# Dunni3/keypoint-diffusion

Measured on AMD Instinct MI355X. Metric: denoising steps/sec, higher is better.
Workload: dtype f32; 1 GPU; egnn_all_atom dynamics (6 EGNN layers, hidden 256, update_kp_feat; fixed receptor encoder), batch of 64 synthetic 300-atom pockets / 25-atom ligands per GPU, T=500, seeded random-init weights, every step taken from the t=T ligand state; batch_per_gpu=64, n_rec=300, n_lig=25, parallelism=dp1

## Files before the change

include/kpd.h:

```cpp
#ifndef KPD_H
#define KPD_H

#include <stdint.h>

#ifdef __cplusplus
extern "C" {
#endif

typedef enum kpd_status {
    KPD_OK = 0,
    KPD_ERR_INVALID = -1,
    KPD_ERR_CAPACITY = -2,
    KPD_ERR_WEIGHTS = -3,
    KPD_ERR_HIP = -4,
    KPD_ERR_STATE = -5
} kpd_status;

const char *kpd_last_error(void);
int kpd_version(void);
int kpd_build_flags(void);

typedef struct kpd_batch {
    int32_t B;
    int32_t n_lig, n_kp;
// ... 16 lines not shown
    int32_t *ll_src, *ll_dst, *ll_rowptr;
    int32_t *kl_src, *kl_dst, *kl_rowptr;
    int32_t *lk_src, *lk_dst, *lk_rowptr;
    int32_t *ll_per_graph;
    int32_t *counts;
} kpd_lig_graph;

kpd_status kpd_build_lig_graph(const kpd_batch *batch, float ll_cutoff, int32_t ll_k, float kl_cutoff,
                               int32_t kl_k, const kpd_lig_graph *out, void *stream);

typedef struct kpd_egnn_config {
    int32_t atom_nf, rec_nf;
    int32_t n_layers, hidden_nf;
    int32_t use_tanh, norm, update_kp_feat;
    float message_norm;
    int32_t ll_k, kl_k;
    float ll_cutoff, kl_cutoff;
    float coords_range;
} kpd_egnn_config;

typedef struct kpd_egnn kpd_egnn;

kpd_status kpd_egnn_create(const kpd_egnn_config *cfg, kpd_egnn **out);
void kpd_egnn_destroy(kpd_egnn *m);
kpd_status kpd_egnn_load_weight(kpd_egnn *m, const char *name, const float *w_dev,
                                const int64_t *shape, int32_t ndim, void *stream);
kpd_status kpd_egnn_commit(kpd_egnn *m);
kpd_status kpd_egnn_reserve(kpd_egnn *m, int32_t max_B, int32_t max_n_lig, int32_t max_n_kp,
                            int32_t max_n_kk, int32_t max_lig_per_graph, int32_t max_kp_per_graph);
kpd_status kpd_egnn_forward(kpd_egnn *m, const kpd_batch *batch, const float *t_dev,
                            float *eps_h_dev, float *eps_x_dev, void *stream);
kpd_status kpd_egnn_debug_state(kpd_egnn *m, const char *what, float *out_dev, int64_t n_floats,
                                void *stream);
kpd_status kpd_egnn_profile(kpd_egnn *m, int32_t enable);
kpd_status kpd_egnn_profile_read(kpd_egnn *m, double *total_ms, int32_t *launches);
kpd_status kpd_egnn_last_counts(kpd_egnn *m, int32_t out[8], void *stream);

typedef struct kpd_egnn_trainer kpd_egnn_trainer;
kpd_status kpd_egnn_trainer_create(const kpd_egnn_config *cfg, kpd_egnn_trainer **out);
void kpd_egnn_trainer_destroy(kpd_egnn_trainer *t);
kpd_status kpd_egnn_trainer_bind(kpd_egnn_trainer *t, const char *name, const float *weight_dev, float *grad_dev,
                                 const int64_t *shape, int32_t ndim);
kpd_status kpd_egnn_trainer_reserve(kpd_egnn_trainer *t, int32_t max_B, int32_t max_n_lig, int32_t max_n_kp,
                                    int32_t max_n_kk, int32_t max_lig_per_graph, int32_t max_kp_per_graph);
kpd_status kpd_egnn_trainer_forward(kpd_egnn_trainer *t, const kpd_batch *batch, const float *t_dev, float *eps_h_dev,
                                    float *eps_x_dev, void *stream);
kpd_status kpd_egnn_trainer_backward(kpd_egnn_trainer *t, const float *d_eps_h, const float *d_eps_x, float *d_lig_h,
                                     float *d_lig_x, float *d_kp_h, float *d_kp_x, void *stream);
kpd_status kpd_egnn_trainer_profile(kpd_egnn_trainer *t, int32_t enable);
kpd_status kpd_egnn_trainer_profile_read(kpd_egnn_trainer *t, double total_ms[2], int32_t launches[2], double edges[2]);

typedef struct kpd_gvp_config {
    int32_t n_lig_scalars, n_kp_scalars;
    int32_t vector_size;
    int32_t n_convs, n_hidden_scalars;
    int32_t update_kp;
    int32_t message_norm_mode;
    float message_norm;
    int32_t ll_k, kl_k;
    float ll_cutoff, kl_cutoff;
    int32_t n_message_gvps, n_update_gvps, n_noise_gvps;
} kpd_gvp_config;

typedef struct kpd_gvp kpd_gvp;

kpd_status kpd_gvp_create(const kpd_gvp_config *cfg, kpd_gvp **out);
// ... 273 lines not shown
```

keypoint-diffusion_amd/csrc/egnn.hip:

```cpp
#include <string.h>

#include <map>
#include <set>
#include <string>
#include <vector>

#include "egnn_kernels.h"
#include "egnn_wide.h"
#include "mfma_core.h"

using namespace kpd;

namespace {

struct LayerW {
    float *wp_e[4], *wx_e[4], *b_e[4], *wr_e[4], *watt[4];
    float *wp_c[4], *wx_c[4], *b_c[4], *wr_c[4], *w3[4];
    void *wh_e[4], *wh_c[4];
    void *chh_p[2][NSLOT];
    void *wh_a[2], *wh_b[2], *wh_2[2];
    float *wp_p[2][NSLOT], *wx_p[2][NSLOT], *b_p[2][NSLOT];
    float *ch_p[2][NSLOT], *wcol_p[2][NSLOT];
    float *wp_a[2], *wx_a[2], *wp_b[2], *wx_b[2], *b0[2], *wp_2[2], *wx_2[2], *b2[2], *ln_w[2], *ln_b[2];
};
// ... 33 lines not shown
struct kpd_egnn {
    kpd_egnn_config cfg;
    int n_et;
    int n_upd;
    bool rec_identity;
    Arena warena, ws;
    std::vector<LayerW> L;
    float *le_W0, *le_b0, *le_W1t, *le_b1;
    float *re_W0, *re_b0, *re_W1t, *re_b1;
    float *de_W0, *de_b0, *de_W1, *de_b1;
    std::set<std::string> expected, loaded;
    bool committed = false;
    int debug_layers = -1;
    bool f16_ok = true;
    float *widen_buf = nullptr;
    int *widen_map = nullptr;
    size_t widen_floats = 0, widen_ints = 0;
    int gemm_mode = 0;
    bool f32_only = false;
    int prune_last = 1;
    bool prof_on = false;
    std::vector<hipEvent_t> prof_ev;
    size_t prof_used = 0;

    int cap_B = 0, cap_lig = 0, cap_kp = 0, cap_kk = 0, cap_ll = 0, cap_kl = 0, cap_maxlig = 0, cap_maxkp = 0;
    int tile_cap = 0, tiles_et_cap[4] = {0, 0, 0, 0};
    float *h[2], *x[2], *P[2];
    float *hn_main[4], *hn_cont[4], *xn_main[4], *xn_cont[4];
    int *bidx[2];
    float *z[2];
    int *meta, *ll_deg, *ll_off, *kl_off, *kl_pg;
    kpd_lig_graph lg;
    int kp_table = 1;
    int tab_rows = 0;
    bool last_table = false;
    int *rowmap = nullptr, *kp_ok = nullptr;
    float *tab_in = nullptr;
    int *tab_bidx = nullptr;
    float *hT = nullptr, *PT = nullptr;
    EgnnWide *wide = nullptr;
};

static kpd_status build_weight_arena(kpd_egnn *m) {
    const kpd_egnn_config &c = m->cfg;
    m->warena.poison_at = 2;
    m->L.assign(c.n_layers, LayerW());
    return carve(m->warena, ARENA_TAIL, [&](Carve &A) {
        for (int i = 0; i < c.n_layers; ++i) {
            LayerW &w = m->L[i];
            const std::string pre = "egnn.conv_layers." + std::to_string(i) + ".";
            for (int et = 0; et < m->n_et; ++et) {
                A(w.wp_e[et], WP_FLOATS); A(w.wx_e[et], HS); A(w.b_e[et], HS); A(w.wr_e[et], HS); A(w.watt[et], HS);
                A(w.wp_c[et], WP_FLOATS); A(w.wx_c[et], HS); A(w.b_c[et], HS); A(w.wr_c[et], HS); A(w.w3[et], HS);
                A.as<unsigned short>(w.wh_e[et], WH_HALVES); A.as<unsigned short>(w.wh_c[et], WH_HALVES);
                for (int var = 0; var < 2; ++var) {
                    const int ss = kSrcSlot[et] + var, ds = kDstSlot[et] + var;
                    A(w.wp_p[kSrcNt[et]][ss], WP_FLOATS); A(w.wx_p[kSrcNt[et]][ss], HS);
                    A(w.wp_p[kDstNt[et]][ds], WP_FLOATS); A(w.wx_p[kDstNt[et]][ds], HS); A(w.b_p[kDstNt[et]][ds], HS);
                    A(w.ch_p[kSrcNt[et]][ss], 16 * 4096); A(w.wcol_p[kSrcNt[et]][ss], HS);
                    A(w.ch_p[kDstNt[et]][ds], 16 * 4096); A(w.wcol_p[kDstNt[et]][ds], HS);
                    A.as<unsigned short>(w.chh_p[kSrcNt[et]][ss], CHH_HALVES);
                    A.as<unsigned short>(w.chh_p[kDstNt[et]][ds], CHH_HALVES);
                }
                const std::string e = kEtName[et];
                for (const char *blk : {"edge_mlp.", "coord_mlp."})
                    for (const char *s : {".0.weight", ".0.bias", ".2.weight", ".2.bias"}) m->expected.insert(pre + blk + e + s);
// ... 473 lines not shown
    const int n_layers = m->debug_layers >= 0 ? std::min(m->debug_layers, c.n_layers) : c.n_layers;

    auto slot_mask = [&](int etmask, int nt) {
        int mk = 0;
        for (int et = 0; et < 4; ++et)
            if ((etmask >> et) & 1) {
                if (kSrcNt[et] == nt) mk |= 3 << kSrcSlot[et];
                if (kDstNt[et] == nt) mk |= 3 << kDstSlot[et];
            }
        return mk;
    };
    auto layer_etmask = [&](int li) { return li == n_layers - 1 ? active_last : active; };
    for (int li = 0; li < n_layers; ++li) {
        const LayerW &L = m->L[li];
        {
            {
                ProjPair pp;
                memset(&pp, 0, sizeof(pp));
                for (int nt = 0; nt < 2; ++nt) {
                    ProjArgs &pa = pp.nt[nt];
                    pa.h = m->h[nt]; pa.n = n[nt]; pa.P = m->P[nt];
                    int k = 0;
                    const int mk = slot_mask(layer_etmask(li), nt);
                    for (int s = 0; s < NSLOT; ++s)
                        if (L.wp_p[nt][s] && ((mk >> s) & 1)) {
                            pa.wp[k] = L.wp_p[nt][s]; pa.wx[k] = L.wx_p[nt][s]; pa.bias[k] = L.b_p[nt][s]; pa.slot[k] = s;
                            pa.chain[k] = L.ch_p[nt][s]; pa.wcol[k] = L.wcol_p[nt][s]; pa.chain_h[k] = L.chh_p[nt][s];
                            ++k;
                        }
                    pp.n_slots[nt] = k;
                }
                pp.tiles0 = cdiv(n[0], TM);
                pp.gemm_mode = m->gemm_mode;
                if (kp_tab && li == 0) {
                    ProjPair pk = pp;
                    pk.n_slots[NT_LIG] = 0;
                    pk.skip_if = m->kp_ok;
                    ProjArgs &pa = pp.nt[NT_KP];
                    pa.h = m->hT; pa.n = n_tab; pa.P = m->PT;
                    KPD_TRY(launch_proj_chain(pp, st));
                    KPD_TRY(launch_proj_chain(pk, st));
                } else {
                    KPD_TRY(launch_proj_chain(pp, st));
                }
            }
        }
        EdgeArgs ea;
        memset(&ea, 0, sizeof(ea));
        const bool last = li == n_layers - 1;
        ea.meta = last ? m->meta + 16 : m->meta;
        ea.x[0] = x_cur[0]; ea.x[1] = x_cur[1]; ea.P[0] = m->P[0]; ea.P[1] = m->P[1];
        ea.use_tanh = c.use_tanh; ea.coords_range = c.coords_range;
        ea.tile_rows = tr;
        ea.gemm_mode = tr == TM ? m->gemm_mode : 0;
        for (int et = 0; et < 4; ++et) {
            ea.src[et] = esrc[et]; ea.dst[et] = edst[et];
            ea.src_nt[et] = kSrcNt[et]; ea.dst_nt[et] = kDstNt[et]; ea.src_slot[et] = kSrcSlot[et]; ea.dst_slot[et] = kDstSlot[et];
            ea.wr_e[et] = L.wr_e[et]; ea.wr_c[et] = L.wr_c[et];
            ea.wp_e[et] = L.wp_e[et]; ea.wx_e[et] = L.wx_e[et]; ea.b_e[et] = L.b_e[et];
            ea.wp_c[et] = L.wp_c[et]; ea.wx_c[et] = L.wx_c[et]; ea.b_c[et] = L.b_c[et];
            ea.wh_e[et] = L.wh_e[et]; ea.wh_c[et] = L.wh_c[et];
            ea.watt[et] = L.watt[et]; ea.w3[et] = L.w3[et];
            ea.hn_main[et] = m->hn_main[et]; ea.hn_cont[et] = m->hn_cont[et];
            ea.xn_main[et] = m->xn_main[et]; ea.xn_cont[et] = m->xn_cont[et];
        }
        if (kp_tab && li == 0) { ea.PT = m->PT; ea.rowmap = m->rowmap; ea.kp_ok = m->kp_ok; }
// ... 47 lines not shown
    KPD_TRY(launch_decode(m->h[NT_LIG], m->x[NT_LIG], bt->lig_x, bt->n_lig, c.atom_nf, 2 * c.atom_nf, m->de_W0, m->de_b0,
                          m->de_W1, m->de_b1, eps_h, eps_x, st));
    return KPD_OK;
}

extern "C" kpd_status kpd_egnn_debug_state(kpd_egnn *m, const char *what, float *out, int64_t n_floats, void *stream) {
    KPD_REQUIRE(m && what && out, KPD_ERR_INVALID, "null argument");
    hipStream_t st = static_cast<hipStream_t>(stream);
    if (m->wide) return wide_debug_state(m->wide, what, out, n_floats, st);
    const std::string w(what);
    const float *src = nullptr;
    if (w == "h_lig") src = m->h[0];
    else if (w == "h_kp") src = m->h[1];
    else if (w == "x_lig") src = m->x[0];
    else if (w == "x_kp") src = m->x[1];
    else if (w == "z_lig") src = m->z[0];
    else if (w == "z_kp") src = m->z[1];
    else if (w.size() == 4 && (w.rfind("xnm", 0) == 0 || w.rfind("xnc", 0) == 0 || w.rfind("hnm", 0) == 0 || w.rfind("hnc", 0) == 0) &&
             w[3] >= '0' && w[3] < '4') {
        const int et = w[3] - '0';
        src = w[0] == 'x' ? (w[2] == 'm' ? m->xn_main[et] : m->xn_cont[et]) : (w[2] == 'm' ? m->hn_main[et] : m->hn_cont[et]);
    }
    else if (w == "kp_table_ok") {
        KPD_REQUIRE(n_floats == 1, KPD_ERR_INVALID, "kp_table_ok is one value");
        if (!m->last_table) {
            KPD_HIP(hipMemsetAsync(out, 0, 4, st));
            return KPD_OK;
        }
        src = reinterpret_cast<const float *>(m->kp_ok);
    } else if (w.rfind("kp_table=", 0) == 0) {
        m->kp_table = atoi(w.c_str() + 9);
        return KPD_OK;
    }
    else if (w.rfind("layers=", 0) == 0) {
        m->debug_layers = atoi(w.c_str() + 7);
        return KPD_OK;
    } else if (w.rfind("prune=", 0) == 0) {
        m->prune_last = atoi(w.c_str() + 6);
        return KPD_OK;
    } else if (w.rfind("gemm=", 0) == 0) {
        const std::string v = w.substr(5);
        KPD_REQUIRE(v == "f32" || v == "f16x2", KPD_ERR_INVALID, "gemm mode must be f32 or f16x2");
        KPD_REQUIRE(v == "f32" || !m->f32_only, KPD_ERR_INVALID,
                    "gemm=f16x2: atom_nf = %d / rec_nf = %d (hidden_nf = %d) run the exact fp32 path only; the f16x2 mode covers atom_nf <= 32 "
                    "with rec_nf <= 128 or 256, or the identity keypoint encoder at hidden_nf 256", m->cfg.atom_nf, m->cfg.rec_nf, m->cfg.hidden_nf);
        KPD_REQUIRE(v == "f32" || !m->committed || m->f16_ok, KPD_ERR_WEIGHTS, "%s", F16_RANGE_ERROR);
        m->gemm_mode = v == "f16x2" ? 1 : 0;
        return KPD_OK;
    }
    KPD_REQUIRE(src, KPD_ERR_INVALID, "unknown debug tap '%s'", what);
    KPD_HIP(hipMemcpyAsync(out, src, (size_t)n_floats * 4, hipMemcpyDeviceToDevice, st));
    return KPD_OK;
}

extern "C" kpd_status kpd_egnn_profile(kpd_egnn *m, int32_t enable) {
    KPD_REQUIRE(m, KPD_ERR_INVALID, "null handle");
    KPD_REQUIRE(!m->wide, KPD_ERR_INVALID, "kpd_egnn_profile times the fused edge kernel of hidden_nf <= 256; hidden_nf = %d has none",
                m->cfg.hidden_nf);
    if (enable && m->prof_ev.empty()) {
        m->prof_ev.resize(2 * 8192);
        for (hipEvent_t &e : m->prof_ev) KPD_HIP(hipEventCreate(&e));
    }
    m->prof_on = enable != 0;
    m->prof_used = 0;
    return KPD_OK;
}
// ... 49 lines not shown
```

keypoint-diffusion_amd/csrc/egnn_chain.hip:

```cpp
#include <algorithm>
#include <cstdlib>

#include "chain_core.h"
#include "egnn_kernels.h"

namespace kpd {

namespace {

constexpr int ENT = 16;
constexpr int ECH4 = ENT * 64;

__device__ __forceinline__ float reduce_q(float v) {
    v += __shfl_xor(v, 16);
    v += __shfl_xor(v, 32);
    return v;
}

}

struct ProjWs {
    ProjPair p;
    int blocks0;
    int bpc[2];
    int tpb;
};

constexpr int WS_TILE = 128;
constexpr int WS_W4 = 16 * 8 * 64;
constexpr int WS_LDS_BYTES = WS_W4 * 16 + (128 + 128 + HS) * 4;

__global__ __launch_bounds__(512, 1) void k_proj_ws(ProjWs qa) {
    extern __shared__ __attribute__((aligned(16))) float smem[];
    v4f *W = reinterpret_cast<v4f *>(smem);
    float *s_wcol = smem + WS_W4 * 4, *s_bias = s_wcol + 128, *s_wrow = s_bias + 128;
    const int tid = threadIdx.x, wave = tid >> 6, lane = tid & 63;
    if (qa.p.skip_if && *qa.p.skip_if) return;
    const int which = (int)blockIdx.x >= qa.blocks0 ? 1 : 0;
    const ProjArgs &a = qa.p.nt[which];
    const int local = blockIdx.x - (which ? qa.blocks0 : 0);
    const int combo = local / qa.bpc[which], chunk = local - combo * qa.bpc[which];
    const int s = combo >> 1, hf = combo & 1;
    const int tiles = (a.n + WS_TILE - 1) / WS_TILE;
    const int t0 = chunk * qa.tpb, t1 = min(tiles, t0 + qa.tpb);
    if (t0 >= t1) return;
    {
        const v4f *src = reinterpret_cast<const v4f *>(a.chain[s]);
#pragma unroll
        for (int j = 0; j < WS_W4 / 512; ++j) {
            const int i = tid + 512 * j, ks = i >> 9, rem = i & 511;
            W[i] = src[(size_t)ks * ECH4 + 8 * hf * 64 + rem];
        }
        const float *bias = a.bias[s];
        if (tid < 128) {
            s_wcol[tid] = a.wcol[s][128 * hf + tid];
            s_bias[tid] = bias ? bias[128 * hf + tid] : 0.0f;
        }
        for (int i = tid; i < HS; i += 512) s_wrow[i] = i <= 256 ? a.wx[s][i] : 0.0f;
    }
    __syncthreads();
    const int el = lane & 15, q = lane >> 4;
    const float bias256 = a.bias[s] ? a.bias[s][256] : 0.0f;
    auto load_x = [&](int t, v4f (&x)[ENT], float &x256) {
        const int row = min(t * WS_TILE + 16 * wave + el, a.n - 1);
        const float *hrow = a.h + (size_t)row * HS;
#pragma unroll
        for (int nt = 0; nt < ENT; ++nt) x[nt] = *reinterpret_cast<const v4f *>(hrow + 16 * nt + 4 * q);
        x256 = hrow[256];
    };
    auto store_tile = [&](const v4f (&acc)[8], int row, float out256) {
        if (row >= 0 && row < a.n) {
            float *orow = a.P + ((size_t)row * NSLOT + a.slot[s]) * HS + 128 * hf;
#pragma unroll
            for (int m = 0; m < 8; ++m) *reinterpret_cast<v4f *>(orow + 16 * m + 4 * q) = acc[m];
            if (hf == 0 && q == 0) orow[256] = out256;
        }
    };
    v4f x[ENT], xn[ENT], accp[8];
    float h256, h256n, out256p = 0.0f;
    int rowp = -1;
#pragma unroll
    for (int m = 0; m < 8; ++m) accp[m] = zero4();
    load_x(t0, xn, h256n);
#pragma unroll 1
    for (int t = t0; t < t1; ++t) {
#pragma unroll
        for (int nt = 0; nt < ENT; ++nt)
#pragma unroll
            for (int r = 0; r < 4; ++r) asm volatile("v_mov_b32 %0, %1" : "=v"(x[nt][r]) : "v"(xn[nt][r]));
        asm volatile("v_mov_b32 %0, %1" : "=v"(h256) : "v"(h256n));
        __builtin_amdgcn_sched_barrier(0);
        store_tile(accp, rowp, out256p);
        if (t + 1 < t1) load_x(t + 1, xn, h256n);
        v4f acc[8];
#pragma unroll
        for (int m = 0; m < 8; ++m)
            acc[m] = h256 * *reinterpret_cast<const v4f *>(s_wcol + 16 * m + 4 * q) + *reinterpret_cast<const v4f *>(s_bias + 16 * m + 4 * q);
        float part = 0.0f;
        if (hf == 0) {
#pragma unroll
            for (int nt = 0; nt < ENT; ++nt) {
                const v4f wv = *reinterpret_cast<const v4f *>(s_wrow + 16 * nt + 4 * q);
                part += x[nt][0] * wv[0] + x[nt][1] * wv[1] + x[nt][2] * wv[2] + x[nt][3] * wv[3];
            }
        }
        const v4f *wp = W + lane;
        v4f w[2][4];
#pragma unroll
        for (int m = 0; m < 4; ++m) w[0][m] = wp[m * 64];
#pragma unroll
        for (int b = 0; b < 32; ++b) {
            if (b + 1 < 32) {
#pragma unroll
                for (int m = 0; m < 4; ++m) w[(b + 1) & 1][m] = wp[(4 * (b + 1) + m) * 64];
            }
            __builtin_amdgcn_sched_barrier(0);
            const v4f xin = x[b >> 1];
            const int g = b & 1;
#pragma unroll
            for (int r = 0; r < 4; ++r)
#pragma unroll
                for (int m = 0; m < 4; ++m) acc[4 * g + m] = mfma16(w[b & 1][m][r], xin[r], acc[4 * g + m]);
            __builtin_amdgcn_sched_barrier(0);
        }
        const int row = t * WS_TILE + 16 * wave + el;
        const float out256 = hf == 0 ? reduce_q(part) + bias256 + h256 * s_wrow[256] : 0.0f;
#pragma unroll
        for (int m = 0; m < 8; ++m) accp[m] = acc[m];
        rowp = row;
        out256p = out256;
    }
    store_tile(accp, rowp, out256p);
}

__global__ __launch_bounds__(512, 1) void k_proj_ws_h(ProjWs qa) {
    extern __shared__ __attribute__((aligned(16))) float smem[];
    f32x4 *W = reinterpret_cast<f32x4 *>(smem);
    float *s_wcol = smem + WS_W4 * 4, *s_bias = s_wcol + 128, *s_wrow = s_bias + 128;
    const int tid = threadIdx.x, wave = tid >> 6, lane = tid & 63;
    const int which = (int)blockIdx.x >= qa.blocks0 ? 1 : 0;
    const ProjArgs &a = qa.p.nt[which];
    const int local = blockIdx.x - (which ? qa.blocks0 : 0);
    const int combo = local / qa.bpc[which], chunk = local - combo * qa.bpc[which];
    const int s = combo >> 1, hf = combo & 1;
    const int tiles = (a.n + WS_TILE - 1) / WS_TILE;
    const int t0 = chunk * qa.tpb, t1 = min(tiles, t0 + qa.tpb);
    if (t0 >= t1) return;
    {
        const f32x4 *src = reinterpret_cast<const f32x4 *>(a.chain_h[s]);
#pragma unroll
        for (int j = 0; j < WS_W4 / 512; ++j) {
            const int i = tid + 512 * j, kb = i >> 10, rem = i & 1023;
            W[i] = src[(size_t)(kb * 16 + 8 * hf) * 128 + rem];
        }
        const float *bias = a.bias[s];
        if (tid < 128) {
            s_wcol[tid] = a.wcol[s][128 * hf + tid];
            s_bias[tid] = bias ? bias[128 * hf + tid] : 0.0f;
        }
        for (int i = tid; i < HS; i += 512) s_wrow[i] = i <= 256 ? a.wx[s][i] : 0.0f;
    }
    __syncthreads();
    const int el = lane & 15, q = lane >> 4;
    const float bias256 = a.bias[s] ? a.bias[s][256] : 0.0f;
    auto load_x = [&](int t, v4f (&x)[16], float &x256) {
// ... 50 lines not shown
        }
        v4f acc[8];
#pragma unroll
        for (int m = 0; m < 8; ++m)
            acc[m] = (1.0f / H_UNSCALE) * (h256 * *reinterpret_cast<const v4f *>(s_wcol + 16 * m + 4 * q) + *reinterpret_cast<const v4f *>(s_bias + 16 * m + 4 * q));
        const f32x4 *wp = W + lane;
        f32x4 w[3][4];
#pragma unroll
        for (int i = 0; i < 4; ++i) w[0][i] = wp[i * 64];
#pragma unroll
        for (int b = 0; b < 32; ++b) {
            if (b + 1 < 32) {
#pragma unroll
                for (int i = 0; i < 4; ++i) w[(b + 1) % 3][i] = wp[(4 * (b + 1) + i) * 64];
            }
            __builtin_amdgcn_sched_barrier(0);
            const int kb = b >> 2, m0 = 2 * (b & 3);
            const f32x4 *wb = w[b % 3];
            acc[m0] = __builtin_amdgcn_mfma_f32_16x16x32_f16(as_h8(wb[1]), as_h8(xh[kb]), acc[m0], 0, 0, 0);
            acc[m0 + 1] = __builtin_amdgcn_mfma_f32_16x16x32_f16(as_h8(wb[3]), as_h8(xh[kb]), acc[m0 + 1], 0, 0, 0);
            acc[m0] = __builtin_amdgcn_mfma_f32_16x16x32_f16(as_h8(wb[0]), as_h8(xl[kb]), acc[m0], 0, 0, 0);
            acc[m0 + 1] = __builtin_amdgcn_mfma_f32_16x16x32_f16(as_h8(wb[2]), as_h8(xl[kb]), acc[m0 + 1], 0, 0, 0);
            acc[m0] = __builtin_amdgcn_mfma_f32_16x16x32_f16(as_h8(wb[0]), as_h8(xh[kb]), acc[m0], 0, 0, 0);
            acc[m0 + 1] = __builtin_amdgcn_mfma_f32_16x16x32_f16(as_h8(wb[2]), as_h8(xh[kb]), acc[m0 + 1], 0, 0, 0);
            __builtin_amdgcn_sched_barrier(0);
        }
#pragma unroll
        for (int m = 0; m < 8; ++m) accp[m] = H_UNSCALE * acc[m];
        rowp = row;
    }
    store_tile(accp, rowp);
}

kpd_status launch_proj_chain(const ProjPair &p, hipStream_t st) {
    const int slots = std::max(p.n_slots[0], p.n_slots[1]);
    if (poison_level() >= 1) KPD_TRY(poison_lds(st));
    if (slots == 0) return KPD_OK;
    for (int nt = 0; nt < 2; ++nt)
        for (int s = 0; s < p.n_slots[nt]; ++s)
            KPD_REQUIRE(p.nt[nt].chain[s] && p.nt[nt].wcol[s], KPD_ERR_STATE, "projection slot %d not packed", s);
    KPD_TRY(ensure_dynamic_lds(reinterpret_cast<const void *>(k_proj_ws), WS_LDS_BYTES));
    const int target = cu_count();
    ProjWs q;
    q.p = p;
    int units = 0, tl[2];
    for (int nt = 0; nt < 2; ++nt) {
        tl[nt] = p.n_slots[nt] ? cdiv(p.nt[nt].n, WS_TILE) : 0;
        units += 2 * p.n_slots[nt] * tl[nt];
    }
    if (units == 0) return KPD_OK;
    int blocks[2];
    for (q.tpb = std::max(1, cdiv(units, target));; ++q.tpb) {
        for (int nt = 0; nt < 2; ++nt) {
            q.bpc[nt] = std::max(1, cdiv(tl[nt], q.tpb));
            blocks[nt] = tl[nt] ? 2 * p.n_slots[nt] * q.bpc[nt] : 0;
        }
        if (blocks[0] + blocks[1] <= target || q.tpb >= std::max(tl[0], tl[1])) break;
    }
    q.blocks0 = blocks[0];
    if (p.gemm_mode == 1) {
        KPD_REQUIRE(!p.skip_if, KPD_ERR_INVALID, "projection launch: skip_if is served by the exact mode only");
        for (int nt = 0; nt < 2; ++nt)
            for (int s = 0; s < p.n_slots[nt]; ++s)
                KPD_REQUIRE(p.nt[nt].chain_h[s], KPD_ERR_STATE, "projection slot %d has no f16 planes (f16x2 mode)", s);
        KPD_TRY(ensure_dynamic_lds(reinterpret_cast<const void *>(k_proj_ws_h), WS_LDS_BYTES));
        hipLaunchKernelGGL(k_proj_ws_h, dim3(blocks[0] + blocks[1]), dim3(512), WS_LDS_BYTES, st, q);
        KPD_LAUNCH_CHECK();
        return KPD_OK;
    }
    hipLaunchKernelGGL(k_proj_ws, dim3(blocks[0] + blocks[1]), dim3(512), WS_LDS_BYTES, st, q);
    KPD_LAUNCH_CHECK();
    return KPD_OK;
}

}
```

keypoint-diffusion_amd/csrc/egnn_kernels.h:

```cpp
#pragma once
#include "engine.h"

namespace kpd {

constexpr int NSLOT = 8;
constexpr int ATT_BIAS_AT = 260;
constexpr int BIAS_K = 260;
constexpr int ET_LL = 0, ET_KL = 1, ET_LK = 2, ET_KK = 3;
constexpr int NT_LIG = 0, NT_KP = 1;

constexpr int EDGE_LDS_BYTES = TM * SA * 4 + (TM * 2 + TM + 3 * TM + TM + 3 * TM + 4 * HS + 8 + TM) * 4;
constexpr int EDGE_H_LDS_BYTES = 64 * 280 * 2 * 2 + (TM * 2 + TM + 3 * TM + TM + 3 * TM + 2 * HS + 8) * 4 + 2 * 2 * 272 * 2;

struct ProjArgs {
    const float *h;
    int n;
    float *P;
    const float *wp[NSLOT];
    const float *wx[NSLOT];
    const float *bias[NSLOT];
    int slot[NSLOT];
    const float *chain[NSLOT];
    const float *wcol[NSLOT];
    const void *chain_h[NSLOT];
};

struct ProjPair {
    ProjArgs nt[2];
    int tiles0;
    int n_slots[2];
    int slots_per_block;
    int gemm_mode;
    const int *skip_if;
};

struct EdgeArgs {
    const int *meta;
    const int *src[4];
    const int *dst[4];
    const float *x[2];
    const float *P[2];
    int src_nt[4], dst_nt[4], src_slot[4], dst_slot[4];
    const float *wr_e[4], *wr_c[4];
    const float *wp_e[4], *wx_e[4], *b_e[4];
    const float *wp_c[4], *wx_c[4], *b_c[4];
    const float *watt[4];
    const float *w3[4];
    float *hn_main[4], *hn_cont[4];
    float *xn_main[4], *xn_cont[4];
    int use_tanh;
    float coords_range;
    const void *wh_e[4], *wh_c[4];
    int gemm_mode;
    int tile_rows;
    int split_slots;
    const float *PT;
    const int *rowmap;
    const int *kp_ok;
};

struct EdgeTrainArgs {
    const int *meta;
    const int *src[4];
    const int *dst[4];
    const float *x[2];
    const float *P[2];
    int src_nt[4], dst_nt[4];
// ... 119 lines not shown
```

keypoint-diffusion_amd/hip.py:

```python
import ctypes as C
import os
from typing import Dict, Optional

import torch

_HERE = os.path.dirname(os.path.abspath(__file__))
LIB_PATH = os.environ.get('KPD_LIB') or os.path.join(_HERE, 'csrc', 'libkpd_hip.so')
_lib = None

c_int_p = C.POINTER(C.c_int32)
c_float_p = C.POINTER(C.c_float)


class KpdBatch(C.Structure):
    _fields_ = [('B', C.c_int32), ('n_lig', C.c_int32), ('n_kp', C.c_int32), ('max_lig', C.c_int32),
                ('max_kp', C.c_int32), ('lig_ptr', C.c_void_p), ('kp_ptr', C.c_void_p), ('lig_x', C.c_void_p),
                ('lig_h', C.c_void_p), ('kp_x', C.c_void_p), ('kp_h', C.c_void_p), ('kp_v', C.c_void_p),
                ('n_kk', C.c_int32), ('kk_src', C.c_void_p), ('kk_dst', C.c_void_p), ('kk_rowptr', C.c_void_p)]


class KpdLigGraph(C.Structure):
    _fields_ = [('cap_ll', C.c_int32), ('cap_kl', C.c_int32),
                ('ll_src', C.c_void_p), ('ll_dst', C.c_void_p), ('ll_rowptr', C.c_void_p),
                ('kl_src', C.c_void_p), ('kl_dst', C.c_void_p), ('kl_rowptr', C.c_void_p),
# ... 62 lines not shown
class KpdError(RuntimeError):
    pass


def lib():
    global _lib
    if _lib is not None:
        return _lib
    if not os.path.exists(LIB_PATH):
        raise KpdError(f'{LIB_PATH} not found: the HIP extension must be built first '
                       f'(python -c "import __graft_entry__ as g; g.build()"). There is no CPU fallback.')
    L = C.CDLL(LIB_PATH)
    L.kpd_last_error.restype = C.c_char_p
    L.kpd_version.restype = C.c_int
    L.kpd_build_flags.restype = C.c_int
    for name in EXPORTS:
        getattr(L, name)
    for family, cfg, n_sizes in (('egnn', KpdEgnnConfig, 6), ('gvp', KpdGvpConfig, 6), ('recenc', KpdRecencConfig, 4),
                                 ('recegnn', KpdRecegnnConfig, 4)):
        for prefix in (family, family + '_trainer'):
            fn = lambda name: getattr(L, f'kpd_{prefix}_{name}')
            fn('create').argtypes = [C.POINTER(cfg), C.POINTER(C.c_void_p)]
            fn('destroy').argtypes = [C.c_void_p]
            fn('destroy').restype = None
            fn('reserve').argtypes = [C.c_void_p] + [C.c_int32] * n_sizes
        fn = lambda name: getattr(L, f'kpd_{family}_{name}')
        fn('load_weight').argtypes = [C.c_void_p, C.c_char_p, C.c_void_p, C.POINTER(C.c_int64), C.c_int32, C.c_void_p]
        fn('commit').argtypes = [C.c_void_p]
        fn('trainer_bind').argtypes = [C.c_void_p, C.c_char_p, C.c_void_p, C.c_void_p, C.POINTER(C.c_int64), C.c_int32]
    L.kpd_egnn_forward.argtypes = [C.c_void_p, C.POINTER(KpdBatch), C.c_void_p, C.c_void_p, C.c_void_p, C.c_void_p]
    L.kpd_egnn_debug_state.argtypes = [C.c_void_p, C.c_char_p, C.c_void_p, C.c_int64, C.c_void_p]
    L.kpd_egnn_last_counts.argtypes = [C.c_void_p, C.POINTER(C.c_int32), C.c_void_p]
    L.kpd_egnn_profile.argtypes = [C.c_void_p, C.c_int32]
    L.kpd_egnn_profile_read.argtypes = [C.c_void_p, C.POINTER(C.c_double), C.POINTER(C.c_int32)]
    L.kpd_gvp_forward.argtypes = [C.c_void_p, C.POINTER(KpdBatch), C.c_void_p, C.c_void_p, C.c_void_p, C.c_void_p]
    L.kpd_gvp_debug_state.argtypes = [C.c_void_p, C.c_char_p, C.c_void_p, C.c_int64, C.c_void_p]
    L.kpd_gvp_last_counts.argtypes = [C.c_void_p, C.POINTER(C.c_int32), C.c_void_p]
    L.kpd_gvp_profile.argtypes = [C.c_void_p, C.c_int32]
    L.kpd_gvp_profile_read.argtypes = [C.c_void_p, C.POINTER(C.c_double), C.POINTER(C.c_int32)]
    L.kpd_recenc_forward.argtypes = [C.c_void_p, C.POINTER(KpdRecBatch), C.POINTER(KpdRecOut), C.c_void_p]
    L.kpd_recegnn_forward.argtypes = [C.c_void_p, C.POINTER(KpdRecBatch), C.c_void_p, C.POINTER(KpdRecOut), C.c_void_p, C.c_void_p,
                                      C.c_void_p]
    L.kpd_build_lig_graph.argtypes = [C.POINTER(KpdBatch), C.c_float, C.c_int32, C.c_float, C.c_int32, C.POINTER(KpdLigGraph),
                                      C.c_void_p]
    L.kpd_sample_update.argtypes = [C.c_int32, C.c_void_p, C.c_void_p, C.c_int32] + [C.c_void_p] * 8 + [C.c_int32, C.c_void_p]
    L.kpd_complex_noise.argtypes = [C.c_int32, C.c_void_p, C.c_int32, C.c_void_p, C.c_uint64, C.c_int32, C.c_int32, C.c_void_p,
                                    C.c_void_p]
    L.kpd_step_coefficients.argtypes = [C.c_void_p, C.c_int32, C.c_void_p, C.c_void_p, C.c_int32, C.c_void_p, C.c_void_p]
    L.kpd_inpaint_coefficients.argtypes = [C.c_void_p, C.c_int32, C.c_void_p, C.c_void_p, C.c_int32, C.c_void_p, C.c_void_p]
    L.kpd_sample_update_inpaint.argtypes = [C.c_int32, C.c_void_p, C.c_void_p, C.c_int32] + [C.c_void_p] * 14 + [C.c_int32, C.c_void_p]
    L.kpd_sample_renoise.argtypes = [C.c_int32, C.c_void_p, C.c_void_p, C.c_int32] + [C.c_void_p] * 6 + [C.c_int32, C.c_void_p]
    L.kpd_guided_coefficients.argtypes = [C.c_void_p, C.c_int32, C.c_void_p, C.c_void_p, C.c_int32, C.c_float, C.c_float, C.c_void_p,
                                          C.c_void_p]
    L.kpd_sample_update_guided.argtypes = ([C.c_int32, C.c_void_p, C.c_void_p, C.c_int32] + [C.c_void_p] * 16 +
                                           [C.c_float, C.c_int32, C.c_void_p])
    L.kpd_clash_score.argtypes = [C.c_int32] + [C.c_void_p] * 4 + [C.c_float, C.c_void_p, C.c_void_p]
    L.kpd_egnn_trainer_forward.argtypes = [C.c_void_p, C.POINTER(KpdBatch), C.c_void_p, C.c_void_p, C.c_void_p, C.c_void_p]
    L.kpd_egnn_trainer_backward.argtypes = [C.c_void_p] + [C.c_void_p] * 7
    L.kpd_egnn_trainer_profile.argtypes = [C.c_void_p, C.c_int32]
    L.kpd_egnn_trainer_profile_read.argtypes = [C.c_void_p, C.POINTER(C.c_double), C.POINTER(C.c_int32), C.POINTER(C.c_double)]
    L.kpd_gvp_trainer_forward.argtypes = [C.c_void_p, C.POINTER(KpdBatch), C.c_void_p, C.c_void_p, C.c_void_p, C.c_void_p]
    L.kpd_gvp_trainer_backward.argtypes = [C.c_void_p] + [C.c_void_p] * 8
    L.kpd_gvp_trainer_set_dropout.argtypes = [C.c_void_p, C.c_float, C.c_uint64]
    L.kpd_gvp_trainer_message_path.argtypes = [C.c_void_p, C.POINTER(C.c_int32)]
    L.kpd_wgrad_batch.argtypes = [C.c_int32, C.c_int32, C.POINTER(KpdWgradItem), C.c_void_p, C.c_int64, C.c_void_p]
    L.kpd_adam_step.argtypes = [C.c_void_p, C.c_int32, C.c_int64, C.c_int32, C.c_double, C.c_double, C.c_double, C.c_double, C.c_double, C.c_int64,
# ... 22 lines not shown
    L.kpd_pocket_select.argtypes = [C.c_void_p] * 5 + [C.c_int32, C.c_int32, C.c_void_p, C.c_void_p, C.c_int32, C.c_int32, C.c_float,
                                    C.c_float, C.c_int32] + [C.c_void_p] * 8
    L.kpd_interface_points_scratch_bytes.argtypes = [C.c_int32, C.c_int32, C.c_int32]
    L.kpd_interface_points_scratch_bytes.restype = C.c_int64
    L.kpd_interface_points.argtypes = [C.c_void_p, C.c_void_p, C.c_void_p, C.c_int32, C.c_void_p, C.c_void_p, C.c_int32, C.c_int32,
                                       C.c_float, C.c_float, C.c_int32, C.c_int32] + [C.c_void_p] * 6
    for name in ('kpd_mol_scratch_bytes', 'kpd_sdf_scratch_bytes'):
        getattr(L, name).argtypes = [C.c_int32, C.c_int32]
        getattr(L, name).restype = C.c_int64
    L.kpd_mol_perceive.argtypes = [C.c_void_p] * 3 + [C.c_int32] * 3 + [C.c_void_p, C.c_void_p, C.c_int32] + [C.c_void_p] * 10
    L.kpd_sdf_emit.argtypes = ([C.c_void_p, C.c_void_p, C.c_int32, C.c_int32, C.c_void_p, C.c_int32] + [C.c_void_p] * 5 +
                               [C.c_int32, C.c_void_p, C.c_int32, C.c_void_p, C.c_int64] + [C.c_void_p] * 4)
    L.kpd_mol_keys.argtypes = ([C.c_void_p, C.c_int32, C.c_int32, C.c_void_p, C.c_int32] + [C.c_void_p] * 5 + [C.c_int32, C.c_void_p] +
                               [C.c_int32] * 4 + [C.c_void_p] * 5)
    L.kpd_fp_diversity.argtypes = [C.c_void_p, C.c_void_p, C.c_int32, C.c_int32, C.c_void_p, C.c_int32] + [C.c_void_p] * 4
    L.kpd_relax_defaults.argtypes = [C.POINTER(KpdRelaxParams)]
    L.kpd_relax_defaults.restype = None
    L.kpd_relax.argtypes = ([C.c_void_p, C.c_void_p, C.c_int32, C.c_int32, C.c_int32, C.c_void_p, C.c_int32] + [C.c_void_p] * 4 +
                            [C.c_int32] + [C.c_void_p] * 4 + [C.c_int32] * 3 + [C.c_void_p, C.POINTER(KpdRelaxParams)] + [C.c_void_p] * 4)
    L.kpd_vina_defaults.argtypes = [C.POINTER(KpdVinaParams)]
    L.kpd_vina_defaults.restype = None
    L.kpd_vina_pocket_types.argtypes = [C.c_void_p] * 3 + [C.c_int32] * 2 + [C.c_void_p] * 3
    L.kpd_vina_score.argtypes = ([C.c_void_p, C.c_void_p, C.c_int32, C.c_int32, C.c_int32, C.c_void_p, C.c_int32] + [C.c_void_p] * 5 +
                                 [C.c_int32] + [C.c_void_p] * 6 + [C.c_int32] * 3 + [C.c_void_p, C.POINTER(KpdVinaParams)] +
                                 [C.c_void_p] * 6)
    _lib = L
    return L


EXPORTS = [
    'kpd_last_error', 'kpd_version', 'kpd_build_flags', 'kpd_build_lig_graph',
    'kpd_egnn_create', 'kpd_egnn_destroy', 'kpd_egnn_load_weight', 'kpd_egnn_commit', 'kpd_egnn_reserve',
    'kpd_egnn_forward', 'kpd_egnn_debug_state', 'kpd_egnn_last_counts', 'kpd_egnn_profile',
    'kpd_egnn_profile_read', 'kpd_sample_update', 'kpd_step_coefficients', 'kpd_complex_noise',
    'kpd_inpaint_coefficients', 'kpd_sample_update_inpaint', 'kpd_sample_renoise',
    'kpd_guided_coefficients', 'kpd_sample_update_guided', 'kpd_clash_score',
    'kpd_gvp_create', 'kpd_gvp_destroy', 'kpd_gvp_load_weight', 'kpd_gvp_commit', 'kpd_gvp_reserve',
    'kpd_gvp_forward', 'kpd_gvp_debug_state', 'kpd_gvp_profile', 'kpd_gvp_profile_read', 'kpd_gvp_last_counts',
    'kpd_recenc_create', 'kpd_recenc_destroy', 'kpd_recenc_load_weight', 'kpd_recenc_commit', 'kpd_recenc_reserve',
    'kpd_recenc_forward',
    'kpd_recegnn_create', 'kpd_recegnn_destroy', 'kpd_recegnn_load_weight', 'kpd_recegnn_commit', 'kpd_recegnn_reserve',
    'kpd_recegnn_forward',
    'kpd_xyz_scratch_bytes', 'kpd_xyz_emit', 'kpd_rec_graph_scratch_bytes', 'kpd_build_rec_graph',
    'kpd_egnn_trainer_create', 'kpd_egnn_trainer_destroy', 'kpd_egnn_trainer_bind', 'kpd_egnn_trainer_reserve',
    'kpd_egnn_trainer_forward', 'kpd_egnn_trainer_backward', 'kpd_egnn_trainer_profile', 'kpd_egnn_trainer_profile_read', 'kpd_gvp_trainer_last_counts',
    'kpd_gvp_trainer_message_path', 'kpd_wgrad_batch', 'kpd_adam_step',
    'kpd_gvp_trainer_create', 'kpd_gvp_trainer_destroy', 'kpd_gvp_trainer_bind', 'kpd_gvp_trainer_reserve',
    'kpd_gvp_trainer_forward', 'kpd_gvp_trainer_backward', 'kpd_gvp_trainer_set_dropout', 'kpd_dropout_mask',
    'kpd_recenc_trainer_create', 'kpd_recenc_trainer_destroy', 'kpd_recenc_trainer_bind', 'kpd_recenc_trainer_set_dropout',
    'kpd_recenc_trainer_reserve', 'kpd_recenc_trainer_forward', 'kpd_recenc_trainer_backward',
    'kpd_recegnn_trainer_create', 'kpd_recegnn_trainer_destroy', 'kpd_recegnn_trainer_bind', 'kpd_recegnn_trainer_reserve',
    'kpd_recegnn_trainer_forward', 'kpd_recegnn_trainer_backward', 'kpd_ot_emd_uniform', 'kpd_sgemm',
    'kpd_dist_hinge',
    'kpd_pocket_scratch_bytes', 'kpd_pocket_select', 'kpd_interface_points_scratch_bytes', 'kpd_interface_points',
    'kpd_mol_scratch_bytes', 'kpd_mol_perceive', 'kpd_sdf_scratch_bytes', 'kpd_sdf_emit',
    'kpd_mol_keys', 'kpd_fp_diversity', 'kpd_relax_defaults', 'kpd_relax',
    'kpd_vina_defaults', 'kpd_vina_pocket_types', 'kpd_vina_score',
]


def check(status: int):
    if status != 0:
        raise KpdError(f'kpd status {status}: {lib().kpd_last_error().decode()}')


def _stream() -> int:
    return torch.cuda.current_stream().cuda_stream
# ... 1027 lines not shown
```

Measured before the change: 157.4 steps/s.

## Load-balance projection GEMM work across workgroups with chunk-level partitioning

Replaces the fixed tiles-per-block split of the exact-mode projection kernel with a host-computed partition of 16-row chunks. Each workgroup may now span up to two (slot, half) segments, and the partition charges an estimated weight-reload cost per segment so work evens out across CUs. A remainder path handles chunk counts that are not a multiple of eight, using per-wave unit MFMAs. The cost is extra kernel complexity, a second weight load into LDS in some workgroups, and a larger kernel argument struct; the f16 mode keeps the old split.

After: 158.7 steps/s (median of 6 runs). No clear change (+0.8%).

```diff
diff --git a/include/kpd.h b/include/kpd.h
--- a/include/kpd.h
+++ b/include/kpd.h
@@ -72,6 +72,8 @@
                             float *eps_h_dev, float *eps_x_dev, void *stream);
 kpd_status kpd_egnn_debug_state(kpd_egnn *m, const char *what, float *out_dev, int64_t n_floats,
                                 void *stream);
+int32_t kpd_proj_partition(const int32_t n_rows[2], const int32_t n_slots[2], int32_t workgroups, int32_t balance,
+                           int32_t *start_out, int32_t cap);
 kpd_status kpd_egnn_profile(kpd_egnn *m, int32_t enable);
 kpd_status kpd_egnn_profile_read(kpd_egnn *m, double *total_ms, int32_t *launches);
 kpd_status kpd_egnn_last_counts(kpd_egnn *m, int32_t out[8], void *stream);
diff --git a/keypoint-diffusion_amd/csrc/egnn.hip b/keypoint-diffusion_amd/csrc/egnn.hip
--- a/keypoint-diffusion_amd/csrc/egnn.hip
+++ b/keypoint-diffusion_amd/csrc/egnn.hip
@@ -89,6 +89,7 @@
     int *meta, *ll_deg, *ll_off, *kl_off, *kl_pg;
     kpd_lig_graph lg;
     int kp_table = 1;
+    int proj_balance = 1;
     int tab_rows = 0;
     bool last_table = false;
     int *rowmap = nullptr, *kp_ok = nullptr;
@@ -628,6 +629,7 @@
                 }
                 pp.tiles0 = cdiv(n[0], TM);
                 pp.gemm_mode = m->gemm_mode;
+                pp.balance = m->proj_balance;
                 if (kp_tab && li == 0) {
                     ProjPair pk = pp;
                     pk.n_slots[NT_LIG] = 0;
@@ -741,6 +743,10 @@
         m->kp_table = atoi(w.c_str() + 9);
         return KPD_OK;
     }
+    else if (w.rfind("proj_balance=", 0) == 0) {
+        m->proj_balance = atoi(w.c_str() + 13);
+        return KPD_OK;
+    }
     else if (w.rfind("layers=", 0) == 0) {
         m->debug_layers = atoi(w.c_str() + 7);
         return KPD_OK;
diff --git a/keypoint-diffusion_amd/csrc/egnn_chain.hip b/keypoint-diffusion_amd/csrc/egnn_chain.hip
--- a/keypoint-diffusion_amd/csrc/egnn_chain.hip
+++ b/keypoint-diffusion_amd/csrc/egnn_chain.hip
@@ -1,5 +1,6 @@
 #include <algorithm>
 #include <cstdlib>
+#include <type_traits>
 
 #include "chain_core.h"
 #include "egnn_kernels.h"
@@ -30,21 +31,37 @@
 constexpr int WS_W4 = 16 * 8 * 64;
 constexpr int WS_LDS_BYTES = WS_W4 * 16 + (128 + 128 + HS) * 4;
 
-__global__ __launch_bounds__(512, 1) void k_proj_ws(ProjWs qa) {
+constexpr int WS_MAX_WG = 320;
+struct ProjWsList {
+    ProjPair p;
+    int chunks[2];
+    int len0;
+    int start[WS_MAX_WG + 1];
+};
+
+__global__ __launch_bounds__(512, 1) void k_proj_ws(ProjWsList qa) {
     extern __shared__ __attribute__((aligned(16))) float smem[];
     v4f *W = reinterpret_cast<v4f *>(smem);
     float *s_wcol = smem + WS_W4 * 4, *s_bias = s_wcol + 128, *s_wrow = s_bias + 128;
-    const int tid = threadIdx.x, wave = tid >> 6, lane = tid & 63;
+    const int tid0 = threadIdx.x;
+    const int wave = __builtin_amdgcn_readfirstlane(tid0 >> 6);
     if (qa.p.skip_if && *qa.p.skip_if) return;
-    const int which = (int)blockIdx.x >= qa.blocks0 ? 1 : 0;
+    const int hi = qa.start[blockIdx.x + 1];
+    int pos = qa.start[blockIdx.x];
+#pragma unroll 1
+    for (int sg = 0; sg < 2; ++sg) {
+    int tid = tid0;
+    asm volatile("" : "+v"(tid));
+    const int lane = tid & 63;
+    const int which = pos >= qa.len0 ? 1 : 0;
     const ProjArgs &a = qa.p.nt[which];
-    const int local = blockIdx.x - (which ? qa.blocks0 : 0);
-    const int combo = local / qa.bpc[which], chunk = local - combo * qa.bpc[which];
+    const int cpc = qa.chunks[which], rel = pos - (which ? qa.len0 : 0);
+    const int combo = rel / cpc, c0 = rel - combo * cpc;
+    const int nc = min(hi - pos, cpc - c0);
     const int s = combo >> 1, hf = combo & 1;
-    const int tiles = (a.n + WS_TILE - 1) / WS_TILE;
-    const int t0 = chunk * qa.tpb, t1 = min(tiles, t0 + qa.tpb);
-    if (t0 >= t1) return;
-    {
+    pos += nc;
+    if (sg) __syncthreads();
+    if (nc > 0) {
         const v4f *src = reinterpret_cast<const v4f *>(a.chain[s]);
 #pragma unroll
         for (int j = 0; j < WS_W4 / 512; ++j) {
@@ -59,10 +76,11 @@
         for (int i = tid; i < HS; i += 512) s_wrow[i] = i <= 256 ? a.wx[s][i] : 0.0f;
     }
     __syncthreads();
+    if (nc <= 0) continue;
     const int el = lane & 15, q = lane >> 4;
     const float bias256 = a.bias[s] ? a.bias[s][256] : 0.0f;
-    auto load_x = [&](int t, v4f (&x)[ENT], float &x256) {
-        const int row = min(t * WS_TILE + 16 * wave + el, a.n - 1);
+    auto load_x = [&](int chunk, v4f (&x)[ENT], float &x256) {
+        const int row = min(16 * chunk + el, a.n - 1);
         const float *hrow = a.h + (size_t)row * HS;
 #pragma unroll
         for (int nt = 0; nt < ENT; ++nt) x[nt] = *reinterpret_cast<const v4f *>(hrow + 16 * nt + 4 * q);
@@ -76,14 +94,18 @@
             if (hf == 0 && q == 0) orow[256] = out256;
         }
     };
-    v4f x[ENT], xn[ENT], accp[8];
-    float h256, h256n, out256p = 0.0f;
+    v4f x[ENT], xn[ENT];
+    float h256, h256n;
+    const int t1 = nc >> 3, k_rem = nc & 7;
+    if (t1 > 0) {
+    v4f accp[8];
+    float out256p = 0.0f;
     int rowp = -1;
 #pragma unroll
     for (int m = 0; m < 8; ++m) accp[m] = zero4();
-    load_x(t0, xn, h256n);
+    load_x(c0 + wave, xn, h256n);
 #pragma unroll 1
-    for (int t = t0; t < t1; ++t) {
+    for (int t = 0; t < t1; ++t) {
 #pragma unroll
         for (int nt = 0; nt < ENT; ++nt)
 #pragma unroll
@@ -91,7 +113,7 @@
         asm volatile("v_mov_b32 %0, %1" : "=v"(h256) : "v"(h256n));
         __builtin_amdgcn_sched_barrier(0);
         store_tile(accp, rowp, out256p);
-        if (t + 1 < t1) load_x(t + 1, xn, h256n);
+        if (t + 1 < t1) load_x(c0 + 8 * (t + 1) + wave, xn, h256n);
         v4f acc[8];
 #pragma unroll
         for (int m = 0; m < 8; ++m)
@@ -123,7 +145,7 @@
                 for (int m = 0; m < 4; ++m) acc[4 * g + m] = mfma16(w[b & 1][m][r], xin[r], acc[4 * g + m]);
             __builtin_amdgcn_sched_barrier(0);
         }
-        const int row = t * WS_TILE + 16 * wave + el;
+        const int row = 16 * (c0 + 8 * t + wave) + el;
         const float out256 = hf == 0 ? reduce_q(part) + bias256 + h256 * s_wrow[256] : 0.0f;
 #pragma unroll
         for (int m = 0; m < 8; ++m) accp[m] = acc[m];
@@ -131,6 +153,63 @@
         out256p = out256;
     }
     store_tile(accp, rowp, out256p);
+    }
+    if (k_rem > 0) {
+        const int cr = c0 + 8 * t1, u0 = wave * k_rem, cA = u0 >> 3;
+        const int nA = min(k_rem, 8 * (cA + 1) - u0), nB = k_rem - nA;
+        int tid_r = tid0;
+        asm volatile("" : "+v"(tid_r));
+        const v4f *wl = W + (tid_r & 63);
+        const int q4 = (tid_r >> 2) & 12;
+        load_x(cr + cA, x, h256);
+        if (nB > 0) load_x(cr + cA + 1, xn, h256n);
+        auto units = [&](auto n_c, const v4f (&xb)[ENT], float hb, int chunk, int u) {
+            constexpr int N = decltype(n_c)::value;
+            int f[N];
+            v4f acc[N];
+#pragma unroll
+            for (int i = 0; i < N; ++i) {
+                f[i] = 16 * ((u + i) & 7) + q4;
+                acc[i] = hb * *reinterpret_cast<const v4f *>(s_wcol + f[i]) + *reinterpret_cast<const v4f *>(s_bias + f[i]);
+            }
+#pragma unroll
+            for (int ks = 0; ks < ENT; ++ks) {
+                v4f wv[N];
+#pragma unroll
+                for (int i = 0; i < N; ++i) wv[i] = wl[(8 * ks + ((u + i) & 7)) * 64];
+#pragma unroll
+                for (int r = 0; r < 4; ++r)
+#pragma unroll
+                    for (int i = 0; i < N; ++i) acc[i] = mfma16(wv[i][r], xb[ks][r], acc[i]);
+            }
+            const int row = 16 * chunk + el;
+            if (row < a.n) {
+                float *orow = a.P + ((size_t)row * NSLOT + a.slot[s]) * HS + 128 * hf;
+#pragma unroll
+                for (int i = 0; i < N; ++i) *reinterpret_cast<v4f *>(orow + f[i]) = acc[i];
+            }
+        };
+        auto group = [&](const v4f (&xb)[ENT], float hb, int chunk, int u, int n) {
+            if (hf == 0 && (u & 7) == 0) {
+                float part = 0.0f;
+#pragma unroll
+                for (int nt = 0; nt < ENT; ++nt) {
+                    const v4f wv = *reinterpret_cast<const v4f *>(s_wrow + 16 * nt + 4 * q);
+                    part += xb[nt][0] * wv[0] + xb[nt][1] * wv[1] + xb[nt][2] * wv[2] + xb[nt][3] * wv[3];
+                }
+                const float out256 = reduce_q(part) + bias256 + hb * s_wrow[256];
+                const int row = 16 * chunk + el;
+                if (q == 0 && row < a.n) a.P[((size_t)row * NSLOT + a.slot[s]) * HS + 256] = out256;
+            }
+            int i = 0;
+#pragma unroll 1
+            for (; i + 2 <= n; i += 2) units(std::integral_constant<int, 2>(), xb, hb, chunk, u + i);
+            if (i < n) units(std::integral_constant<int, 1>(), xb, hb, chunk, u + i);
+        };
+        group(x, h256, cr + cA, u0, nA);
+        if (nB > 0) group(xn, h256n, cr + cA + 1, u0 + nA, nB);
+    }
+    }
 }
 
 __global__ __launch_bounds__(512, 1) void k_proj_ws_h(ProjWs qa) {
@@ -247,6 +326,79 @@
     store_tile(accp, rowp);
 }
 
+static int tiles_per_wg(const int tl[2], const int combos[2], int target, int bpc[2], int blocks[2]) {
+    const int units = combos[0] * tl[0] + combos[1] * tl[1];
+    for (int tpb = std::max(1, cdiv(units, target));; ++tpb) {
+        for (int nt = 0; nt < 2; ++nt) {
+            bpc[nt] = std::max(1, cdiv(tl[nt], tpb));
+            blocks[nt] = tl[nt] ? combos[nt] * bpc[nt] : 0;
+        }
+        if (blocks[0] + blocks[1] <= target || tpb >= std::max(tl[0], tl[1])) return tpb;
+    }
+}
+
+constexpr double WS_RELOAD_CHUNKS = 3.5;
+
+int proj_partition(const int chunks[2], const int combos[2], int target, int balance, int *start, int cap) {
+    target = std::max(1, std::min(target, cap));
+    const long total = (long)combos[0] * chunks[0] + (long)combos[1] * chunks[1];
+    const int n_combos = combos[0] + combos[1];
+    if (total == 0) { start[0] = 0; return 0; }
+    if (!balance) {
+        const int tl[2] = {combos[0] ? cdiv(chunks[0], 8) : 0, combos[1] ? cdiv(chunks[1], 8) : 0};
+        int bpc[2], blocks[2], g = 0, base = 0;
+        const int tpb = tiles_per_wg(tl, combos, target, bpc, blocks);
+        for (int nt = 0; nt < 2; ++nt)
+            for (int ci = 0; ci < combos[nt]; ++ci, base += chunks[nt])
+                for (int c = 0; c < chunks[nt] && g < cap; c += 8 * tpb) start[g++] = base + c;
+        start[g] = (int)total;
+        return g;
+    }
+    const double R = WS_RELOAD_CHUNKS;
+    auto walk = [&](double S) {
+        int g = 0, nt = combos[0] ? 0 : 1, ci = 0, off = 0, pos = 0;
+        double used = 0.0;
+        while (nt < 2) {
+            if (g >= target) return -1;
+            start[g] = pos;
+            double budget = std::min((g + 1) * S - used, S + 1.0);
+            for (int segs = 0; segs < 2 && nt < 2; ++segs) {
+                const int L = chunks[nt], rem = L - off, avail = (int)std::floor(budget - R);
+                if (avail < 1 && segs) break;
+                int take;
+                if (rem <= avail) take = rem;
+                else if (L < 8) {
+                    if (segs) break;
+                    take = rem;
+                } else take = std::max(avail, 1);
+                off += take; pos += take; budget -= R + take; used += R + take;
+                if (off < L) break;
+                off = 0;
+                if (++ci == combos[nt]) { ci = 0; nt = (nt == 0 && combos[1]) ? 1 : 2; }
+            }
+            ++g;
+        }
+        start[g] = pos;
+        return g;
+    };
+    for (double S = std::max(R + 1.0, (total + R * (n_combos + target - 1)) / target);; S += 0.25) {
+        const int g = walk(S);
+        if (g >= 0) return g;
+    }
+}
+
+extern "C" int32_t kpd_proj_partition(const int32_t n_rows[2], const int32_t n_slots[2], int32_t workgroups, int32_t balance,
+                                      int32_t *start_out, int32_t cap) {
+    if (!n_rows || !n_slots || !start_out || workgroups < 1 || cap < 2) return -1;
+    int chunks[2], combos[2];
+    for (int nt = 0; nt < 2; ++nt) {
+        if (n_slots[nt] < 0 || n_slots[nt] > NSLOT || n_rows[nt] < 0) return -1;
+        combos[nt] = n_rows[nt] > 0 ? 2 * n_slots[nt] : 0;
+        chunks[nt] = std::max(1, cdiv(n_rows[nt], 16));
+    }
+    return proj_partition(chunks, combos, workgroups, balance, start_out, std::min(cap - 1, WS_MAX_WG));
+}
+
 kpd_status launch_proj_chain(const ProjPair &p, hipStream_t st) {
     const int slots = std::max(p.n_slots[0], p.n_slots[1]);
     if (poison_level() >= 1) KPD_TRY(poison_lds(st));
@@ -256,34 +408,34 @@
             KPD_REQUIRE(p.nt[nt].chain[s] && p.nt[nt].wcol[s], KPD_ERR_STATE, "projection slot %d not packed", s);
     KPD_TRY(ensure_dynamic_lds(reinterpret_cast<const void *>(k_proj_ws), WS_LDS_BYTES));
     const int target = cu_count();
+    int tl[2], combos[2];
+    for (int nt = 0; nt < 2; ++nt) {
+        combos[nt] = p.nt[nt].n > 0 ? 2 * p.n_slots[nt] : 0;
+        tl[nt] = combos[nt] ? cdiv(p.nt[nt].n, WS_TILE) : 0;
+    }
+    if (combos[0] * tl[0] + combos[1] * tl[1] == 0) return KPD_OK;
+    if (p.gemm_mode != 1) {
+        ProjWsList q;
+        q.p = p;
+        for (int nt = 0; nt < 2; ++nt) q.chunks[nt] = std::max(1, cdiv(p.nt[nt].n, 16));
+        q.len0 = combos[0] * q.chunks[0];
+        const int grid = proj_partition(q.chunks, combos, target, p.balance, q.start, WS_MAX_WG);
+        for (int g = grid + 1; g <= WS_MAX_WG; ++g) q.start[g] = q.start[grid];
+        hipLaunchKernelGGL(k_proj_ws, dim3(grid), dim3(512), WS_LDS_BYTES, st, q);
+        KPD_LAUNCH_CHECK();
+        return KPD_OK;
+    }
     ProjWs q;
     q.p = p;
-    int units = 0, tl[2];
-    for (int nt = 0; nt < 2; ++nt) {
-        tl[nt] = p.n_slots[nt] ? cdiv(p.nt[nt].n, WS_TILE) : 0;
-        units += 2 * p.n_slots[nt] * tl[nt];
-    }
-    if (units == 0) return KPD_OK;
     int blocks[2];
-    for (q.tpb = std::max(1, cdiv(units, target));; ++q.tpb) {
-        for (int nt = 0; nt < 2; ++nt) {
-            q.bpc[nt] = std::max(1, cdiv(tl[nt], q.tpb));
-            blocks[nt] = tl[nt] ? 2 * p.n_slots[nt] * q.bpc[nt] : 0;
-        }
-        if (blocks[0] + blocks[1] <= target || q.tpb >= std::max(tl[0], tl[1])) break;
-    }
+    q.tpb = tiles_per_wg(tl, combos, target, q.bpc, blocks);
     q.blocks0 = blocks[0];
-    if (p.gemm_mode == 1) {
-        KPD_REQUIRE(!p.skip_if, KPD_ERR_INVALID, "projection launch: skip_if is served by the exact mode only");
-        for (int nt = 0; nt < 2; ++nt)
-            for (int s = 0; s < p.n_slots[nt]; ++s)
-                KPD_REQUIRE(p.nt[nt].chain_h[s], KPD_ERR_STATE, "projection slot %d has no f16 planes (f16x2 mode)", s);
-        KPD_TRY(ensure_dynamic_lds(reinterpret_cast<const void *>(k_proj_ws_h), WS_LDS_BYTES));
-        hipLaunchKernelGGL(k_proj_ws_h, dim3(blocks[0] + blocks[1]), dim3(512), WS_LDS_BYTES, st, q);
-        KPD_LAUNCH_CHECK();
-        return KPD_OK;
-    }
-    hipLaunchKernelGGL(k_proj_ws, dim3(blocks[0] + blocks[1]), dim3(512), WS_LDS_BYTES, st, q);
+    KPD_REQUIRE(!p.skip_if, KPD_ERR_INVALID, "projection launch: skip_if is served by the exact mode only");
+    for (int nt = 0; nt < 2; ++nt)
+        for (int s = 0; s < p.n_slots[nt]; ++s)
+            KPD_REQUIRE(p.nt[nt].chain_h[s], KPD_ERR_STATE, "projection slot %d has no f16 planes (f16x2 mode)", s);
+    KPD_TRY(ensure_dynamic_lds(reinterpret_cast<const void *>(k_proj_ws_h), WS_LDS_BYTES));
+    hipLaunchKernelGGL(k_proj_ws_h, dim3(blocks[0] + blocks[1]), dim3(512), WS_LDS_BYTES, st, q);
     KPD_LAUNCH_CHECK();
     return KPD_OK;
 }
diff --git a/keypoint-diffusion_amd/csrc/egnn_kernels.h b/keypoint-diffusion_amd/csrc/egnn_kernels.h
--- a/keypoint-diffusion_amd/csrc/egnn_kernels.h
+++ b/keypoint-diffusion_amd/csrc/egnn_kernels.h
@@ -32,7 +32,10 @@
     int slots_per_block;
     int gemm_mode;
     const int *skip_if;
+    int balance;
 };
+
+int proj_partition(const int chunks[2], const int combos[2], int target, int balance, int *start, int cap);
 
 struct EdgeArgs {
     const int *meta;
diff --git a/keypoint-diffusion_amd/hip.py b/keypoint-diffusion_amd/hip.py
--- a/keypoint-diffusion_amd/hip.py
+++ b/keypoint-diffusion_amd/hip.py
@@ -118,6 +118,7 @@
     L.kpd_egnn_debug_state.argtypes = [C.c_void_p, C.c_char_p, C.c_void_p, C.c_int64, C.c_void_p]
     L.kpd_egnn_last_counts.argtypes = [C.c_void_p, C.POINTER(C.c_int32), C.c_void_p]
     L.kpd_egnn_profile.argtypes = [C.c_void_p, C.c_int32]
+    L.kpd_proj_partition.argtypes = [C.POINTER(C.c_int32), C.POINTER(C.c_int32), C.c_int32, C.c_int32, C.POINTER(C.c_int32), C.c_int32]
     L.kpd_egnn_profile_read.argtypes = [C.c_void_p, C.POINTER(C.c_double), C.POINTER(C.c_int32)]
     L.kpd_gvp_forward.argtypes = [C.c_void_p, C.POINTER(KpdBatch), C.c_void_p, C.c_void_p, C.c_void_p, C.c_void_p]
     L.kpd_gvp_debug_state.argtypes = [C.c_void_p, C.c_char_p, C.c_void_p, C.c_int64, C.c_void_p]
@@ -206,7 +207,7 @@
     'kpd_last_error', 'kpd_version', 'kpd_build_flags', 'kpd_build_lig_graph',
     'kpd_egnn_create', 'kpd_egnn_destroy', 'kpd_egnn_load_weight', 'kpd_egnn_commit', 'kpd_egnn_reserve',
     'kpd_egnn_forward', 'kpd_egnn_debug_state', 'kpd_egnn_last_counts', 'kpd_egnn_profile',
-    'kpd_egnn_profile_read', 'kpd_sample_update', 'kpd_step_coefficients', 'kpd_complex_noise',
+    'kpd_egnn_profile_read', 'kpd_proj_partition', 'kpd_sample_update', 'kpd_step_coefficients', 'kpd_complex_noise',
     'kpd_inpaint_coefficients', 'kpd_sample_update_inpaint', 'kpd_sample_renoise',
     'kpd_guided_coefficients', 'kpd_sample_update_guided', 'kpd_clash_score',
     'kpd_gvp_create', 'kpd_gvp_destroy', 'kpd_gvp_load_weight', 'kpd_gvp_commit', 'kpd_gvp_reserve',
```
